# ActiveVisionLab/CrossScore

Measured on AMD Instinct MI355X. Metric: query-images/sec at 518x518, 5 ref views, bs=8; score-map MAE vs ref, higher is better.
Workload: dtype fp16

## Files before the change

### crossscore_amd/csrc/panel.hip

```cpp
#include "cs_common.h"
#include "panel_shared.h"
#include <atomic>
#include <stdlib.h>
#include <type_traits>
#include <utility>

namespace {

constexpr int PC = 384;
constexpr int PF = 1536;
constexpr int NT = PC / 32;
constexpr int KS = PC / 16;
constexpr int NSL = PF / 32;
constexpr int FRAG = 1024;
constexpr int CHUNK = 24 * FRAG;
constexpr int TICK = 48 * FRAG;
constexpr int OUT_CHUNKS = KS / 2;
constexpr int LAGT = 2;
constexpr int NTICK = NSL + LAGT;
constexpr int PAD_TICKS = 1;
constexpr int PANEL_ROWS = 128;
constexpr int LDS_RING = 0;
constexpr int LDS_X = 3 * CHUNK;
constexpr int XREC = 6 * FRAG;
constexpr int LDS_OF = LDS_X + 3 * 4 * 4 * FRAG;
constexpr int LDS_XF = 2 * TICK;
constexpr int LDS_HB = LDS_OF;
constexpr int HB_PAIR = 6 * FRAG;
constexpr int HB_RAW = 2 * FRAG;
constexpr int LDS_B1 = LDS_OF + 3 * 4 * 2 * FRAG;
constexpr int LDS_BV = LDS_B1 + PF * 4;
constexpr int LDS_BYTES = LDS_BV + 2 * PC * 4;
constexpr int ST_ROW = 784;
constexpr int ST_PAIR = 32 * ST_ROW;

#ifdef CS_PANEL_ABLATE
__device__ unsigned long long g_panel_dbg[64 * 8 * 16];
#define CS_STAMP(k) do { if (blockIdx.x < 64 && lane == 0) { \
    __builtin_amdgcn_sched_barrier(0); g_panel_dbg[(blockIdx.x * 8 + wv) * 16 + (k)] = __builtin_amdgcn_s_memtime(); __builtin_amdgcn_sched_barrier(0); } } while (0)
#define CS_STAMP_RT(k) do { if (blockIdx.x < 64 && lane == 0) g_panel_dbg[(blockIdx.x * 8 + wv) * 16 + (k)] = __builtin_amdgcn_s_memrealtime(); } while (0)
__device__ unsigned long long g_panel_bar[4 * 8 * 16 * 2];
#define CS_BAR_STAMP(v, k) do { if (blockIdx.x < 4 && (v) >= 40 && (v) < 56 && (threadIdx.x & 63) == 0) { \
    __builtin_amdgcn_sched_barrier(0); g_panel_bar[((blockIdx.x * 8 + wv) * 16 + ((v) - 40)) * 2 + (k)] = __builtin_amdgcn_s_memtime(); __builtin_amdgcn_sched_barrier(0); } } while (0)
#else
#define CS_STAMP(k) do { } while (0)
#define CS_STAMP_RT(k) do { } while (0)
#define CS_BAR_STAMP(v, k) do { } while (0)
#endif

template <bool OUTPROJ, int ABL = 0, bool BF = false>
__global__ __launch_bounds__(512, 2) void cs_panel_kernel(CsPanelParams p) {
  extern __shared__ __attribute__((aligned(16))) char smem[];
  const int tid = threadIdx.x;
  const int lane = tid & 63;
  const int wv = __builtin_amdgcn_readfirstlane(tid >> 6);
  const bool is_a = wv < 4;
  const int pair = wv & 3;
  const int j = lane & 31, h = lane >> 5;
  const int row0 = blockIdx.x * PANEL_ROWS + pair * 32;
  const size_t row = (size_t)min(row0 + j, p.M - 1);
  constexpr int NOUT = OUTPROJ ? OUT_CHUNKS : 0;
  constexpr size_t IMG_MLP = (size_t)NOUT * CHUNK;
  const unsigned lds0 = (unsigned)(size_t)CS_LDS_PTR(smem);
  const unsigned lane16 = lane * 16;
  const unsigned xoff = (unsigned)row * (PC * 4) + 64 * h;
  const unsigned ooff = (unsigned)row * (PC * 2) + 16 * h;

  int u_next = 0;
  auto out_unit_issue = [&](int c) {
    const int slot = c % 3;
    const unsigned dst = lds0 + LDS_RING + slot * CHUNK + pair * 6 * FRAG;
    const char* s6 = reinterpret_cast<const char*>(p.img) + (size_t)c * CHUNK + pair * 6 * FRAG + lane16;
    dma_piece<0>(s6, dst); dma_piece<FRAG>(s6, dst); dma_piece<2 * FRAG>(s6, dst); dma_piece<3 * FRAG>(s6, dst);
    dma_piece<0>(s6 + 4 * FRAG, dst + 4 * FRAG); dma_piece<FRAG>(s6 + 4 * FRAG, dst + 4 * FRAG);
    const unsigned dx = lds0 + LDS_X + (slot * 4 + pair) * XREC;
    const char* sx = reinterpret_cast<const char*>(p.x) + (size_t)(xoff + c * 128);
    dma_piece<0>(sx, dx); dma_piece<0>(sx + 16, dx + FRAG); dma_piece<0>(sx + 32, dx + 2 * FRAG); dma_piece<0>(sx + 48, dx + 3 * FRAG);
    const unsigned dof = dx + 4 * FRAG;
    const char* so = reinterpret_cast<const char*>(p.attn_o) + (size_t)(ooff + c * 64);
    dma_piece<0>(so, dof); dma_piece<0>(so + 32, dof + FRAG);
  };
  int pend_u = 0;
  bool pend = false;
  auto issue_piece = [&](auto K_) {
    constexpr int K = decltype(K_)::value;
    const unsigned dst = lds0 + LDS_RING + (pend_u & 3) * CHUNK + (pair * 6 + (K & ~3)) * FRAG;
    const char* s = reinterpret_cast<const char*>(p.img) + (IMG_MLP + (size_t)pend_u * CHUNK + (pair * 6 + (K & ~3)) * FRAG) + lane16;
    dma_piece<(K & 3) * FRAG>(s, dst);
  };
  auto tick_issue_all = [&](int t) {
    sfor<12>([&](auto K_) {
      constexpr int K = decltype(K_)::value % 6, HF = decltype(K_)::value / 6;
      const unsigned dst = lds0 + LDS_RING + (t & 1) * TICK + HF * CHUNK + (pair * 6 + (K & ~3)) * FRAG;
      const char* s = reinterpret_cast<const char*>(p.img) + (IMG_MLP + (size_t)t * TICK + HF * CHUNK + (pair * 6 + (K & ~3)) * FRAG) + lane16;
      dma_piece<(K & 3) * FRAG>(s, dst);
    });
  };
  unsigned long long tw_drain = 0, tw_vm = 0, tw_bar = 0;
  auto transition = [&](auto ISA_) -> unsigned {
    constexpr bool ISA = decltype(ISA_)::value;
    CS_SB();
    unsigned long long ta = 0, tb = 0, tc = 0, td = 0;
    if constexpr (ABL & 64) { asm volatile("s_memtime %0" : "=s"(ta)::"memory"); }
    asm volatile("s_waitcnt lgkmcnt(0)" ::: "memory");
    if constexpr (ABL & 64) { asm volatile("s_memtime %0\n\ts_waitcnt lgkmcnt(0)" : "=s"(tb)::"memory"); }
    if constexpr (ISA) {
      if (u_next + 1 < NOUT) CS_VMCNT(12);
      else CS_VMCNT(0);
    } else {
      CS_VMCNT(0);
    }
    if constexpr (ABL & 64) { asm volatile("s_memtime %0\n\ts_waitcnt lgkmcnt(0)" : "=s"(tc)::"memory"); }
    if constexpr (!(ABL & 16)) __builtin_amdgcn_s_barrier();
    if constexpr (ABL & 64) {
      asm volatile("s_memtime %0\n\ts_waitcnt lgkmcnt(0)" : "=s"(td)::"memory");
      tw_drain += tb - ta; tw_vm += tc - tb; tw_bar += td - tc;
    }
    asm volatile("" ::: "memory");
    if (u_next + 2 < NOUT) {
      if constexpr (ISA && OUTPROJ) out_unit_issue(u_next + 2);
    } else if (u_next + 1 >= NOUT) {
      const int t = u_next + 1 - NOUT;
      if constexpr (ISA) {
        if (t < 2) tick_issue_all(t);
      }
    }
    const unsigned base = lds0 + LDS_RING + lane16 + (u_next < NOUT ? (u_next % 3) * CHUNK : ((u_next - NOUT) & 1) * TICK);
    ++u_next;
    CS_SB();
    return base;
  };
  using TA = std::true_type;
  using TB = std::false_type;
  h16x8_t w[6];

  if (is_a) {
    CS_STAMP_RT(8); CS_STAMP(0);
    for (int i = tid; i < PF / 4; i += 256)
      reinterpret_cast<f32x4_t*>(smem + LDS_B1)[i] = reinterpret_cast<const f32x4_t*>(p.b1)[i];
    if (tid < PC / 4) {
      reinterpret_cast<f32x4_t*>(smem + LDS_BV)[tid] = OUTPROJ ? reinterpret_cast<const f32x4_t*>(p.bo)[tid] : f32x4_t{0.f, 0.f, 0.f, 0.f};
      reinterpret_cast<f32x4_t*>(smem + LDS_BV + PC * 4)[tid] = reinterpret_cast<const f32x4_t*>(p.b2)[tid];
    }
    asm volatile("s_waitcnt vmcnt(0) lgkmcnt(0)" ::: "memory");
    if constexpr (OUTPROJ) { out_unit_issue(0); out_unit_issue(1); }
    else tick_issue_all(0);
    unsigned cur = transition(TA{});
    CS_STAMP(1);
    for (int c = 0; c < NOUT; ++c) cur = transition(TA{});
    CS_STAMP(2);
    h16x8_t xf[KS];
    const unsigned r_addr = lds0 + LDS_XF + pair * 12 * FRAG + lane16;
    __builtin_amdgcn_s_barrier();
    sfor<12>([&](auto F_) { lds_read1<decltype(F_)::value * FRAG>(r_addr, xf[decltype(F_)::value]); });
    CS_LGKM(0);
    __builtin_amdgcn_s_barrier();
    __builtin_amdgcn_s_barrier();
    sfor<12>([&](auto F_) { lds_read1<decltype(F_)::value * FRAG>(r_addr, xf[12 + decltype(F_)::value]); });
    CS_LGKM(0);
    CS_STAMP(3);

    f32x16_t acE, acO;
    const unsigned bias_addr = lds0 + LDS_B1 + 64 * h;
    f32x4_t bb[4];
    auto read_bias = [&](int t) {
      const unsigned a = bias_addr + t * 128;
      lds_read_f4<0>(a, bb[0]); lds_read_f4<16>(a, bb[1]); lds_read_f4<32>(a, bb[2]); lds_read_f4<48>(a, bb[3]);
    };
    const unsigned hb_base = lds0 + LDS_HB + pair * HB_PAIR + lane16;
    const unsigned ring = lds0 + LDS_RING + lane16;
    unsigned xa[4] = {0u, 0u, 0u, 0u}, xb[4];
    PkGelu pg;
    const PkGeluK kk = pk_gelu_consts();
    auto boundary = [&](auto FC1_, int v) {
      CS_SB();
      if constexpr (!decltype(FC1_)::value) { asm volatile("s_waitcnt lgkmcnt(0)" ::: "memory"); }
      CS_BAR_STAMP(v, 0);
      CS_VMCNT(6);
      if constexpr (!(ABL & 16)) __builtin_amdgcn_s_barrier();
      asm volatile("" ::: "memory");
      CS_BAR_STAMP(v, 1);
      pend_u = v + 3;
      pend = v >= 1 && v + 3 < 2 * NTICK && !(ABL & 2);
      CS_SB();
    };
    auto tick = [&](auto FC1_, f32x16_t& acc, const f32x16_t& act, int hb_slot, int t, int t_next, bool hb_write) {
      constexpr bool FC1 = decltype(FC1_)::value;
      sfor<24>([&](auto M_) {
        constexpr int M = decltype(M_)::value;
        if constexpr (M == 6) boundary(FC1_, 2 * t);
        if constexpr (M == 18) {
          boundary(FC1_, 2 * t + 1);
          cur = ring + ((t + 1) & 1) * TICK;
          if constexpr (FC1) read_bias(t_next);
        }
        if constexpr ((M >= 6 && M < 12) || M >= 18) {
          if (pend) issue_piece(IC<(M >= 18 ? M - 18 : M - 6)>{});
        }
        if constexpr (M == 1) {
          if constexpr (!FC1) asm volatile("s_nop 15\n\ts_nop 15\n\ts_nop 15\n\ts_nop 15\n\ts_nop 15\n\ts_nop 15" ::: "memory");
#pragma unroll
          for (int i = 0; i < 4; ++i) xa[i] = pack_h16x2(act[2 * i], act[2 * i + 1]);
        }
        if constexpr (!BF) {
          if constexpr (M == 4) {
#pragma unroll
            for (int i = 0; i < 4; ++i) xb[i] = pack_h16x2(act[8 + 2 * i], act[9 + 2 * i]);
          }
          if constexpr (M == 5) {
            if (hb_write) lds_write16<HB_RAW>(hb_base + hb_slot * (2 * FRAG), u32x4_t{xb[0], xb[1], xb[2], xb[3]});
          }
        } else {
          if constexpr (M == 5) {
            if (hb_write) {
              lds_write16<HB_RAW>(hb_base + hb_slot * (2 * FRAG), __builtin_bit_cast(u32x4_t, f32x4_t{act[8], act[9], act[10], act[11]}));
              lds_write16<HB_RAW + FRAG>(hb_base + hb_slot * (2 * FRAG), __builtin_bit_cast(u32x4_t, f32x4_t{act[12], act[13], act[14], act[15]}));
            }
          }
        }
        if constexpr (FC1) {
          CS_LGKM(5);
          if constexpr (M == 0) {
            f32x16_t b16;
#pragma unroll
            for (int q = 0; q < 4; ++q)
#pragma unroll
              for (int i = 0; i < 4; ++i) b16[4 * q + i] = bb[q][i];
            if constexpr (ABL & 4) acc = b16;
            else acc = mfma_32x32x16<BF>(w[0], xf[0], b16);
          } else if constexpr (!(ABL & 4)) {
            acc = mfma_32x32x16<BF>(w[M % 6], xf[M], acc);
          }
          constexpr int F = (M + 6) % 24;
          if constexpr (!(ABL & 32)) lds_read1<((F / 12) * 24 + F % 12) * FRAG>(cur, w[M % 6]);
        }
        if constexpr (M >= 2 && M < 12 && !(ABL & 1)) {
          constexpr int B0 = M < 3 ? 0 : (M < 8 ? M - 1 : M);
          const float a8[8] = {act[0], act[1], act[2], act[3], act[4], act[5], act[6], act[7]};
          pk_gelu_op<B0, BF>(pg, xa, kk, a8);
          if constexpr (M == 2 || M == 7) pk_gelu_op<B0 + 1, BF>(pg, xa, kk, a8);
        }
        if constexpr (M == 11) { if (hb_write) lds_write16<0>(hb_base + hb_slot * FRAG, u32x4_t{xa[0], xa[1], xa[2], xa[3]}); }
        CS_SB();
      });
    };
    read_bias(0);
    sfor<6>([&](auto F_) { lds_read1<decltype(F_)::value * FRAG>(cur, w[decltype(F_)::value]); });
#pragma unroll
    for (int i = 0; i < 16; ++i) acO[i] = 0.f;
    for (int t = 0; t < NSL; t += 2) {
      tick(std::true_type{}, acE, acO, 1, t, t + 1, t > 0);
      tick(std::true_type{}, acO, acE, 0, t + 1, min(t + 2, NSL - 1), true);
    }
    CS_STAMP(4);
    CS_LGKM(0);
    tick(std::false_type{}, acE, acO, 1, NSL, 0, true);
    CS_VMCNT(0);
    if constexpr (!(ABL & 16)) __builtin_amdgcn_s_barrier();
    CS_STAMP(5);
    {
      const unsigned st_addr = lds0 + pair * ST_PAIR + (lane >> 4) * ST_ROW + (lane & 15) * 16;
      const int r_in = lane >> 4;
      auto drain = [&](char* gbase, size_t row_bytes) {
#pragma unroll
        for (int rg = 0; rg < 8; ++rg) {
          f32x4_t v[3];
          lds_read_f4<0>(st_addr + rg * 4 * ST_ROW, v[0]);
          lds_read_f4<256>(st_addr + rg * 4 * ST_ROW, v[1]);
          lds_read_f4<512>(st_addr + rg * 4 * ST_ROW, v[2]);
          CS_LGKM(0);
          const int r = rg * 4 + r_in;
          if (row0 + r < p.M) {
            char* g = gbase + (size_t)r * row_bytes + (lane & 15) * 16;
            *reinterpret_cast<f32x4_t*>(g) = v[0];
            *reinterpret_cast<f32x4_t*>(g + 256) = v[1];
            *reinterpret_cast<f32x4_t*>(g + 512) = v[2];
          }
        }
      };
      char* xg = reinterpret_cast<char*>(p.x + (size_t)row0 * PC);
      __builtin_amdgcn_s_barrier();
      __builtin_amdgcn_s_barrier();
      drain(xg, PC * 4);
      __builtin_amdgcn_s_barrier();
      __builtin_amdgcn_s_barrier();
      drain(xg + 768, PC * 4);
      __builtin_amdgcn_s_barrier();
      if (p.u_out) {
        __builtin_amdgcn_s_barrier();
        drain(reinterpret_cast<char*>(p.u_out + (size_t)row0 * PC), PC * 2);
      }
    }
    asm volatile("s_waitcnt vmcnt(0)" ::: "memory");
    CS_STAMP_RT(9);
#ifdef CS_PANEL_ABLATE
    if (blockIdx.x < 64 && lane == 0) { unsigned long long* d = g_panel_dbg + (blockIdx.x * 8 + wv) * 16; d[10] = tw_drain; d[11] = tw_vm; d[12] = tw_bar; }
#endif
    return;
  }

  CS_STAMP_RT(8); CS_STAMP(0);
  f32x16_t acc2[NT];
  const unsigned bv_addr = lds0 + LDS_BV + 64 * (fresh_lane() >> 5);
  unsigned cur = transition(TB{});
  CS_STAMP(1);
  auto add_bias = [&](auto T_, auto INIT_, int which) {
    constexpr int T = decltype(T_)::value;
    f32x4_t b4[4];
    const unsigned a = bv_addr + which * (PC * 4);
    lds_read_f4<T * 128>(a, b4[0]); lds_read_f4<T * 128 + 16>(a, b4[1]); lds_read_f4<T * 128 + 32>(a, b4[2]); lds_read_f4<T * 128 + 48>(a, b4[3]);
    CS_LGKM(0);
#pragma unroll
    for (int q = 0; q < 4; ++q)
#pragma unroll
      for (int i = 0; i < 4; ++i) acc2[T][4 * q + i] = (decltype(INIT_)::value ? 0.f : acc2[T][4 * q + i]) + b4[q][i];
  };
  if constexpr (OUTPROJ) {
    sfor<NT>([&](auto T_) { add_bias(T_, std::true_type{}, 0); });
    const unsigned xs_addr = lds0 + LDS_X + pair * XREC + lane16;
    h16x8_t of[2];
    lds_read1<4 * FRAG>(xs_addr, of[0]);
    lds_read1<5 * FRAG>(xs_addr, of[1]);
    sfor<6>([&](auto F_) { lds_read1<decltype(F_)::value * FRAG>(cur, w[decltype(F_)::value]); });
    int slot_x = 0;
    sfor<OUT_CHUNKS>([&](auto C_) {
      constexpr int C = decltype(C_)::value;
      f32x4_t xs;
      sfor<24>([&](auto M_) {
        constexpr int M = decltype(M_)::value;
        if constexpr (M >= 13 && M <= 16) {
          constexpr int Q = M - 13;
          CS_LGKM(1);
#pragma unroll
          for (int i = 0; i < 4; ++i) acc2[C][4 * Q + i] += xs[i];
          CS_SB();
        }
        if constexpr (M >= 12 && M <= 15) lds_read_f4<(M - 12) * FRAG>(xs_addr + slot_x * (4 * XREC), xs);
        if constexpr (M == 18) {
          cur = transition(TB{});
          slot_x = slot_x + 1 >= 3 ? 0 : slot_x + 1;
          if constexpr (C + 1 < OUT_CHUNKS) lds_read1<4 * FRAG>(xs_addr + slot_x * (4 * XREC), of[0]);
        }
        if constexpr (M == 0 && C > 0) lds_read1<5 * FRAG>(xs_addr + slot_x * (4 * XREC), of[1]);
        CS_LGKM(5);
        constexpr int T = M % 12;
        acc2[T] = mfma_32x32x16<BF>(w[M % 6], of[M / 12], acc2[T]);
        if constexpr (M < 18) lds_read1<(M + 6) * FRAG>(cur, w[M % 6]);
        else lds_read1<(M - 18) * FRAG>(cur, w[M % 6]);
        CS_SB();
      });
    });
    CS_LGKM(0);
  } else {
    const float* xr = p.x + row * PC + 16 * h;
#pragma unroll
    for (int T = 0; T < NT; ++T)
#pragma unroll
      for (int q = 0; q < 4; ++q) {
        const f32x4_t v = *reinterpret_cast<const f32x4_t*>(xr + 32 * T + 4 * q);
#pragma unroll
        for (int i = 0; i < 4; ++i) acc2[T][4 * q + i] = v[i];
      }
    asm volatile("s_waitcnt vmcnt(0)" ::: "memory");
  }
  CS_STAMP(2);

  auto row_stats = [&](float& mean, float& rstd) {
    float s = 0.f;
#pragma unroll
    for (int T = 0; T < NT; ++T)
#pragma unroll
      for (int r = 0; r < 16; r += 4) s += (acc2[T][r] + acc2[T][r + 1]) + (acc2[T][r + 2] + acc2[T][r + 3]);
    s = add_other_half(s);
    mean = s * (1.0f / PC);
    float q = 0.f;
#pragma unroll
    for (int T = 0; T < NT; ++T)
#pragma unroll
      for (int r = 0; r < 16; ++r) {
        const float d = acc2[T][r] - mean;
        q = fmaf(d, d, q);
      }
    q = add_other_half(q);
    rstd = 1.0f / sqrtf(q * (1.0f / PC) + p.eps);
  };
  {
    float mean, rstd;
    row_stats(mean, rstd);
    const float nb = -mean * rstd;
    const unsigned r_addr = lds0 + LDS_XF + pair * 12 * FRAG + lane16;
    auto put = [&](auto T_, auto S_) {
      constexpr int T = decltype(T_)::value, S = decltype(S_)::value;
      float v[8];
#pragma unroll
      for (int e = 0; e < 8; ++e) v[e] = fmaf(acc2[T][8 * S + e], rstd, nb);
      lds_write16<((2 * T + S) % 12) * FRAG>(r_addr, pack8<BF>(v));
    };
    sfor<6>([&](auto T_) { put(T_, IC<0>{}); put(T_, IC<1>{}); });
    asm volatile("s_waitcnt lgkmcnt(0)" ::: "memory");
    __builtin_amdgcn_s_barrier();
    __builtin_amdgcn_s_barrier();
    sfor<6>([&](auto T_) { put(IC<6 + decltype(T_)::value>{}, IC<0>{}); put(IC<6 + decltype(T_)::value>{}, IC<1>{}); });
    asm volatile("s_waitcnt lgkmcnt(0)" ::: "memory");
    __builtin_amdgcn_s_barrier();
  }
  sfor<NT>([&](auto T_) { add_bias(T_, std::false_type{}, 1); });
  CS_STAMP(3);

  for (int g = 0; g < 2 * LAGT; ++g) { if constexpr (!(ABL & 16)) __builtin_amdgcn_s_barrier(); }
  const unsigned hb_base = lds0 + LDS_HB + pair * HB_PAIR + lane16;
  int cur_step = TICK;
  h16x8_t hb0;
  u32x4_t hb1;
  f32x4_t rw[2];
  u32x4_t xr;
  unsigned hx[4];
  PkGelu pg;
  const PkGeluK kk = pk_gelu_consts();
  auto fc2_tick = [&](int slice, bool more) {
    sfor<24>([&](auto M_) {
      constexpr int M = decltype(M_)::value;
      if constexpr (M == 6) { CS_SB(); CS_BAR_STAMP(2 * (slice + LAGT), 0); if constexpr (!(ABL & 16)) __builtin_amdgcn_s_barrier(); asm volatile("" ::: "memory"); CS_BAR_STAMP(2 * (slice + LAGT), 1); CS_SB(); }
      if constexpr (M == 18) {
        if (more) {
          CS_SB();
          CS_BAR_STAMP(2 * (slice + LAGT) + 1, 0);
          if constexpr (!(ABL & 16)) __builtin_amdgcn_s_barrier();
          asm volatile("" ::: "memory");
          CS_BAR_STAMP(2 * (slice + LAGT) + 1, 1);
          cur += cur_step;
          cur_step = -cur_step;
          lds_read1<0>(hb_base + ((slice + 1) & 1) * FRAG, hb0);
          if constexpr (BF) {
            lds_read_f4<HB_RAW>(hb_base + ((slice + 1) & 1) * (2 * FRAG), rw[0]);
            lds_read_f4<HB_RAW + FRAG>(hb_base + ((slice + 1) & 1) * (2 * FRAG), rw[1]);
          } else {
            lds_read_u4<HB_RAW>(hb_base + ((slice + 1) & 1) * (2 * FRAG), xr);
          }
          CS_SB();
        }
      }
      CS_LGKM(5);
      if constexpr (ABL & 8) { if constexpr (M == 12) asm volatile("" ::"v"(hb1)); }
      else if constexpr (M < 12) acc2[M % 12] = mfma_32x32x16<BF>(w[M % 6], hb0, acc2[M % 12]);
      else acc2[M % 12] = mfma_32x32x16<BF>(w[M % 6], __builtin_bit_cast(h16x8_t, hb1), acc2[M % 12]);
      constexpr int F = (M + 6) % 24;
      if constexpr (!(ABL & 32)) lds_read1<((F / 12) * 24 + 12 + F % 12) * FRAG>(cur, w[M % 6]);
      if constexpr (M == 0) {
#pragma unroll
        for (int i = 0; i < 4; ++i) {
          if constexpr (BF) hx[i] = pack_h16x2(rw[i >> 1][2 * (i & 1)], rw[i >> 1][2 * (i & 1) + 1]);
          else hx[i] = xr[i];
        }
      }
      if constexpr (M < 12 && !(ABL & 1)) {
        const float a8[8] = {rw[0][0], rw[0][1], rw[0][2], rw[0][3], rw[1][0], rw[1][1], rw[1][2], rw[1][3]};
        pk_gelu_op<M, BF>(pg, hx, kk, a8);
      }
      if constexpr (M == 11) hb1 = u32x4_t{hx[0], hx[1], hx[2], hx[3]};
      CS_SB();
    });
  };
  cur = lds0 + LDS_RING + lane16;
  lds_read1<0>(hb_base, hb0);
  if constexpr (BF) {
    lds_read_f4<HB_RAW>(hb_base, rw[0]);
    lds_read_f4<HB_RAW + FRAG>(hb_base, rw[1]);
  } else {
    lds_read_u4<HB_RAW>(hb_base, xr);
  }
  sfor<6>([&](auto F_) { lds_read1<(12 + decltype(F_)::value) * FRAG>(cur, w[decltype(F_)::value]); });
  for (int sl = 0; sl < NSL - 1; ++sl) fc2_tick(sl, true);
  fc2_tick(NSL - 1, false);
  CS_LGKM(0);
  CS_VMCNT(0);
  CS_STAMP(4);

  {
    const unsigned le = fresh_lane();
    const unsigned st_addr = (unsigned)(size_t)CS_LDS_PTR(smem) + pair * ST_PAIR + (le & 31) * ST_ROW + 64 * (le >> 5);
    auto stage_x = [&](auto HALF_) {
      constexpr int HALF = decltype(HALF_)::value;
      sfor<6>([&](auto T_) {
        constexpr int T = 6 * HALF + decltype(T_)::value;
        sfor<4>([&](auto Q_) {
          constexpr int Q = decltype(Q_)::value;
          lds_write16<decltype(T_)::value * 128 + 16 * Q>(st_addr, __builtin_bit_cast(u32x4_t, f32x4_t{acc2[T][4 * Q], acc2[T][4 * Q + 1], acc2[T][4 * Q + 2], acc2[T][4 * Q + 3]}));
        });
      });
      asm volatile("s_waitcnt lgkmcnt(0)" ::: "memory");
    };
    __builtin_amdgcn_s_barrier();
    stage_x(IC<0>{});
    __builtin_amdgcn_s_barrier();
    float mean = 0.f, rstd = 0.f;
    if (p.u_out) row_stats(mean, rstd);
    __builtin_amdgcn_s_barrier();
    stage_x(IC<1>{});
    __builtin_amdgcn_s_barrier();
    __builtin_amdgcn_s_barrier();
    if (p.u_out) {
      const float nb = -mean * rstd;
      const unsigned su = (unsigned)(size_t)CS_LDS_PTR(smem) + pair * ST_PAIR + (le & 31) * ST_ROW + 32 * (le >> 5);
      sfor<NT>([&](auto T_) {
        constexpr int T = decltype(T_)::value;
        sfor<2>([&](auto Q_) {
          constexpr int Q = decltype(Q_)::value;
          float v[8];
#pragma unroll
          for (int e = 0; e < 8; ++e) v[e] = fmaf(acc2[T][8 * Q + e], rstd, nb);
          lds_write16<T * 64 + 16 * Q>(su, pack8<BF>(v));
        });
      });
      asm volatile("s_waitcnt lgkmcnt(0)" ::: "memory");
      __builtin_amdgcn_s_barrier();
    }
  }
  asm volatile("s_waitcnt vmcnt(0)" ::: "memory");
  CS_STAMP(5); CS_STAMP_RT(9);
#ifdef CS_PANEL_ABLATE
  if (blockIdx.x < 64 && lane == 0) { unsigned long long* d = g_panel_dbg + (blockIdx.x * 8 + wv) * 16; d[10] = tw_drain; d[11] = tw_vm; d[12] = tw_bar; }
#endif
}

__device__ __forceinline__ int panel_perm(int i) { return 16 * ((i >> 2) & 1) + (i & 3) + 4 * (i >> 3); }
template <bool BF>
__global__ __launch_bounds__(256) void cs_panel_pack_kernel(const float* __restrict__ wo, const float* __restrict__ ls1,
                                                            const float* __restrict__ w1, const float* __restrict__ g2,
                                                            const float* __restrict__ w2, const float* __restrict__ ls2,
                                                            h16_t* __restrict__ img) {
  const int nout = wo ? OUT_CHUNKS : 0;
  const long long n_out16 = (long long)nout * (CHUNK / 16);
  const long long total16 = n_out16 + (long long)(NTICK + PAD_TICKS) * (TICK / 16);
  const long long gi = (long long)blockIdx.x * blockDim.x + threadIdx.x;
  if (gi >= total16) return;
  float v[8] = {0.f, 0.f, 0.f, 0.f, 0.f, 0.f, 0.f, 0.f};
  if (gi < n_out16) {
    const int c = (int)(gi / (CHUNK / 16));
    const int within = (int)(gi - (long long)c * (CHUNK / 16));
    const int f = within >> 6, lane = within & 63, i = lane & 31, h = lane >> 5;
    const int ks = 2 * c + f / 12, T = f % 12;
    const int rowi = 32 * T + panel_perm(i);
#pragma unroll
    for (int e = 0; e < 8; ++e) v[e] = wo[(size_t)rowi * PC + 16 * ks + 8 * h + e] * (ls1 ? ls1[rowi] : 1.f);
  } else {
    const long long g2i = gi - n_out16;
    const int t = (int)(g2i / (TICK / 16));
    const int within = (int)(g2i - (long long)t * (TICK / 16));
    const int fpos = within >> 6, lane = within & 63, i = lane & 31, h = lane >> 5;
    const int f = ((fpos % 24) / 12) * 24 + (fpos / 24) * 12 + fpos % 12;
    if (t < NTICK) {
      if (f < 24) {
        if (t < NSL) {
          const int ks = f;
          const int rowi = 32 * t + panel_perm(i);
#pragma unroll
          for (int e = 0; e < 8; ++e) {
            const int col = 32 * (ks >> 1) + 16 * h + 8 * (ks & 1) + e;
            v[e] = w1[(size_t)rowi * PC + col] * (g2 ? g2[col] : 1.f);
          }
        }
      } else if (t >= LAGT) {
        const int tt = t - LAGT, fp = f - 24;
        const int s = fp / 12, T = fp % 12;
        const int rowi = 32 * T + panel_perm(i);
#pragma unroll
        for (int e = 0; e < 8; ++e) {
          const int col = 32 * tt + 16 * h + 8 * s + e;
          v[e] = w2[(size_t)rowi * PF + col] * (ls2 ? ls2[rowi] : 1.f);
        }
      }
    }
  }
  const uint4 o = {pack_o16x2<BF>(v[0], v[1]), pack_o16x2<BF>(v[2], v[3]), pack_o16x2<BF>(v[4], v[5]), pack_o16x2<BF>(v[6], v[7])};
  reinterpret_cast<uint4*>(img)[gi] = o;
}

template <bool OUTPROJ, bool BF>
hipError_t panel_launch_t(const CsPanelParams* p, hipStream_t st) {
  static std::atomic<bool> attr_done[16];
  int dev = 0;
  if (hipGetDevice(&dev) != hipSuccess || dev < 0 || dev >= 16) return hipErrorInvalidDevice;
  if (!attr_done[dev]) {
    hipError_t e = hipFuncSetAttribute(reinterpret_cast<const void*>(cs_panel_kernel<OUTPROJ, 0, BF>), hipFuncAttributeMaxDynamicSharedMemorySize, LDS_BYTES);
    if (e != hipSuccess) return e;
    attr_done[dev] = true;
  }
  const int grid = (p->M + PANEL_ROWS - 1) / PANEL_ROWS;
  hipLaunchKernelGGL((cs_panel_kernel<OUTPROJ, 0, BF>), dim3(grid), dim3(512), LDS_BYTES, st, *p);
  return hipGetLastError();
}

}

extern "C" {

#ifdef CS_PANEL_ABLATE
int cs_panel_debug_read(unsigned long long* dst) { return (int)hipMemcpyFromSymbol(dst, HIP_SYMBOL(g_panel_dbg), sizeof(g_panel_dbg)); }
int cs_panel_bar_read(unsigned long long* dst) { return (int)hipMemcpyFromSymbol(dst, HIP_SYMBOL(g_panel_bar), sizeof(g_panel_bar)); }
#endif

int cs_panel_supported(int C, int mlp_ratio) { return C == PC && mlp_ratio * C == PF; }
size_t cs_panel8_image_bytes(int with_outproj) { return (size_t)(with_outproj ? OUT_CHUNKS : 0) * CHUNK + (size_t)(NTICK + PAD_TICKS) * TICK; }

hipError_t cs_panel_pack_launch(const float* wo, const float* ls1, const float* w1, const float* g2, const float* w2, const float* ls2,
                                h16_t* img, int bf16, hipStream_t st) {
  const int total = (int)(cs_panel8_image_bytes(wo ? 1 : 0) / 16);
  if (bf16) hipLaunchKernelGGL(cs_panel_pack_kernel<true>, dim3((total + 255) / 256), dim3(256), 0, st, wo, ls1, w1, g2, w2, ls2, img);
  else hipLaunchKernelGGL(cs_panel_pack_kernel<false>, dim3((total + 255) / 256), dim3(256), 0, st, wo, ls1, w1, g2, w2, ls2, img);
  return hipGetLastError();
}

const char* cs_panel_check(const CsPanelParams* p) {
  if (!p->x || !p->img || !p->b1 || !p->b2) return "panel: null operand";
  if (p->attn_o && !p->bo) return "panel: the out-projection needs its bias";
  if (p->M <= 0) return "panel: empty shape";
  if ((long long)p->M * PC * 4 >= (1ll << 32)) return "panel: too many rows for 32-bit byte offsets";
  if (((uintptr_t)p->x | (uintptr_t)p->img | (uintptr_t)p->b1 | (uintptr_t)p->b2 | (uintptr_t)p->attn_o | (uintptr_t)p->u_out | (uintptr_t)p->bo) & 15)
    return "panel: operands must be 16-byte aligned";
  return nullptr;
}

hipError_t cs_panel_launch(const CsPanelParams* p, hipStream_t st) {
#ifdef CS_PANEL_ABLATE
  if (const char* e = getenv("CS_PANEL_ABL")) {
    const int abl = atoi(e);
    const int grid = (p->M + PANEL_ROWS - 1) / PANEL_ROWS;
#define CS_ABL_CASE(N) if (abl == N) { \
      (void)hipFuncSetAttribute(reinterpret_cast<const void*>(cs_panel_kernel<true, N>), hipFuncAttributeMaxDynamicSharedMemorySize, LDS_BYTES); \
      hipLaunchKernelGGL((cs_panel_kernel<true, N>), dim3(grid), dim3(512), LDS_BYTES, st, *p); return hipGetLastError(); }
    CS_ABL_CASE(1) CS_ABL_CASE(2) CS_ABL_CASE(3) CS_ABL_CASE(4) CS_ABL_CASE(8) CS_ABL_CASE(12) CS_ABL_CASE(16) CS_ABL_CASE(18) CS_ABL_CASE(32) CS_ABL_CASE(34) CS_ABL_CASE(50) CS_ABL_CASE(64)
#undef CS_ABL_CASE
  }
#endif
  if (p->attn_o) return p->bf16 ? panel_launch_t<true, true>(p, st) : panel_launch_t<true, false>(p, st);
  return p->bf16 ? panel_launch_t<false, true>(p, st) : panel_launch_t<false, false>(p, st);
}

}
```

### crossscore_amd/csrc/panel_shared.h

```cpp
#pragma once
#include "cs_common.h"
#include <type_traits>
#include <utility>

namespace {

constexpr int PANEL_FRAG = 1024;

#define CS_VMCNT(n) asm volatile("s_waitcnt vmcnt(%0)" ::"n"(n) : "memory")
#define CS_SB() __builtin_amdgcn_sched_barrier(0)
#define CS_LGKM(n) do { asm volatile("s_waitcnt lgkmcnt(%0)" ::"n"(n) : "memory"); CS_SB(); } while (0)

template <int V> using IC = std::integral_constant<int, V>;
template <int... Js, class F>
__device__ __forceinline__ void static_for(std::integer_sequence<int, Js...>, F&& f) {
  (f(IC<Js>{}), ...);
}
template <int N, class F>
__device__ __forceinline__ void sfor(F&& f) { static_for(std::make_integer_sequence<int, N>{}, f); }

struct PkGeluK { unsigned nk, c5, c4, c3, c2, c1, c0, vc6; };
__device__ __forceinline__ PkGeluK pk_gelu_consts() {
  PkGeluK k;
  asm volatile("s_mov_b32 %0, 0xb400b400" : "=s"(k.nk));
  asm volatile("s_mov_b32 %0, 0xbd76bd76" : "=s"(k.c5));
  asm volatile("s_mov_b32 %0, 0xb8a3b8a3" : "=s"(k.c4));
  asm volatile("s_mov_b32 %0, 0x3e8a3e8a" : "=s"(k.c3));
  asm volatile("s_mov_b32 %0, 0x394a394a" : "=s"(k.c2));
  asm volatile("s_mov_b32 %0, 0xb52cb52c" : "=s"(k.c1));
  asm volatile("s_mov_b32 %0, 0xb086b086" : "=s"(k.c0));
  asm volatile("v_mov_b32 %0, 0x3a443a44" : "=v"(k.vc6));
  return k;
}
struct PkGelu { unsigned t0, t1, q0, q1, r0, r1; };
template <int B, bool BF>
__device__ __forceinline__ void pk_gelu_block(PkGelu& g, unsigned& x0, unsigned& x1, const PkGeluK& k, float a0, float a1, float a2, float a3) {
  if constexpr (B == 0)
    asm("v_pk_max_f16 %0, %2, %2 neg_lo:[0,1] neg_hi:[0,1]\n\t"
        "v_pk_max_f16 %1, %3, %3 neg_lo:[0,1] neg_hi:[0,1]\n\t"
        "v_pk_fma_f16 %0, %0, %4, 1.0 op_sel_hi:[1,1,0] clamp\n\t"
        "v_pk_fma_f16 %1, %1, %4, 1.0 op_sel_hi:[1,1,0] clamp"
        : "=&v"(g.t0), "=&v"(g.t1) : "v"(x0), "v"(x1), "s"(k.nk));
  else if constexpr (B == 1)
    asm("v_pk_fma_f16 %0, %0, %0, -0.5 op_sel_hi:[1,1,0]\n\t"
        "v_pk_fma_f16 %1, %1, %1, -0.5 op_sel_hi:[1,1,0]\n\t"
        "v_pk_fma_f16 %2, %0, %4, %5\n\t"
        "v_pk_fma_f16 %3, %1, %4, %5"
        : "+v"(g.t0), "+v"(g.t1), "=&v"(g.q0), "=&v"(g.q1) : "v"(k.vc6), "s"(k.c5));
  else if constexpr (B == 2)
    asm("v_pk_fma_f16 %0, %0, %2, %4\n\t"
        "v_pk_fma_f16 %1, %1, %3, %4\n\t"
        "v_pk_fma_f16 %0, %0, %2, %5\n\t"
        "v_pk_fma_f16 %1, %1, %3, %5"
        : "+v"(g.q0), "+v"(g.q1) : "v"(g.t0), "v"(g.t1), "s"(k.c4), "s"(k.c3));
  else if constexpr (B == 3)
    asm("v_pk_fma_f16 %0, %0, %2, %4\n\t"
        "v_pk_fma_f16 %1, %1, %3, %4\n\t"
        "v_pk_fma_f16 %0, %0, %2, %5\n\t"
        "v_pk_fma_f16 %1, %1, %3, %5"
        : "+v"(g.q0), "+v"(g.q1) : "v"(g.t0), "v"(g.t1), "s"(k.c2), "s"(k.c1));
  else if constexpr (B == 4 && BF)
    asm("v_pk_fma_f16 %0, %0, %2, %4\n\t"
        "v_pk_fma_f16 %1, %1, %3, %4"
        : "+v"(g.q0), "+v"(g.q1) : "v"(g.t0), "v"(g.t1), "s"(k.c0));
  else if constexpr (B == 5 && BF) {
    float y0, y1, y2, y3;
    asm("v_max_f32 %2, 0, %6\n\t"
        "v_max_f32 %3, 0, %7\n\t"
        "v_max_f32 %4, 0, %8\n\t"
        "v_max_f32 %5, 0, %9\n\t"
        "v_fma_mix_f32 %2, %10, 1.0, %2 op_sel_hi:[1,0,0]\n\t"
        "v_fma_mix_f32 %3, %10, 1.0, %3 op_sel:[1,0,0] op_sel_hi:[1,0,0]\n\t"
        "v_fma_mix_f32 %4, %11, 1.0, %4 op_sel_hi:[1,0,0]\n\t"
        "v_fma_mix_f32 %5, %11, 1.0, %5 op_sel:[1,0,0] op_sel_hi:[1,0,0]\n\t"
        "v_cvt_pk_bf16_f32 %0, %2, %3\n\t"
        "v_cvt_pk_bf16_f32 %1, %4, %5"
        : "=&v"(x0), "=&v"(x1), "=&v"(y0), "=&v"(y1), "=&v"(y2), "=&v"(y3)
        : "v"(a0), "v"(a1), "v"(a2), "v"(a3), "v"(g.q0), "v"(g.q1));
  } else if constexpr (B == 4)
    asm("v_pk_fma_f16 %0, %0, %4, %6\n\t"
        "v_pk_fma_f16 %1, %1, %5, %6\n\t"
        "v_pk_max_f16 %2, %7, 0 op_sel_hi:[1,0]\n\t"
        "v_pk_max_f16 %3, %8, 0 op_sel_hi:[1,0]"
        : "+v"(g.q0), "+v"(g.q1), "=&v"(g.r0), "=&v"(g.r1) : "v"(g.t0), "v"(g.t1), "s"(k.c0), "v"(x0), "v"(x1));
  else
    asm("v_pk_add_f16 %0, %2, %4\n\t"
        "v_pk_add_f16 %1, %3, %5"
        : "=&v"(x0), "=&v"(x1) : "v"(g.q0), "v"(g.q1), "v"(g.r0), "v"(g.r1));
}
template <int N, bool BF>
__device__ __forceinline__ void pk_gelu_op(PkGelu& g, unsigned (&x)[4], const PkGeluK& k, const float (&a)[8]) {
  if constexpr (N >= 0 && N < 12) {
    constexpr int P = 2 * (N / 6);
    pk_gelu_block<N % 6, BF>(g, x[P], x[P + 1], k, a[2 * P], a[2 * P + 1], a[2 * P + 2], a[2 * P + 3]);
  }
}

__device__ __forceinline__ unsigned fresh_lane() {
  unsigned l;
  asm volatile("v_mbcnt_lo_u32_b32 %0, -1, 0\n\tv_mbcnt_hi_u32_b32 %0, -1, %0" : "=v"(l));
  return l;
}
__device__ __forceinline__ float add_other_half(float x) {
  const auto r = __builtin_amdgcn_permlane32_swap(__float_as_uint(x), __float_as_uint(x), false, false);
  return __uint_as_float(r[0]) + __uint_as_float(r[1]);
}

typedef unsigned u32x4_t __attribute__((ext_vector_type(4)));
template <bool BF>
__device__ __forceinline__ u32x4_t pack8(const float (&v)[8]) {
  return u32x4_t{pack_o16x2<BF>(v[0], v[1]), pack_o16x2<BF>(v[2], v[3]), pack_o16x2<BF>(v[4], v[5]), pack_o16x2<BF>(v[6], v[7])};
}

template <int OFF>
__device__ __forceinline__ void lds_read1(unsigned addr, h16x8_t& w) {
  asm volatile("ds_read_b128 %0, %1 offset:%2" : "=&v"(w) : "v"(addr), "n"(OFF) : "memory");
}
template <int OFF>
__device__ __forceinline__ void lds_read_f4(unsigned addr, f32x4_t& w) {
  asm volatile("ds_read_b128 %0, %1 offset:%2" : "=&v"(w) : "v"(addr), "n"(OFF) : "memory");
}
template <int OFF>
__device__ __forceinline__ void lds_read_u4(unsigned addr, u32x4_t& w) {
  asm volatile("ds_read_b128 %0, %1 offset:%2" : "=&v"(w) : "v"(addr), "n"(OFF) : "memory");
}
template <int OFF>
__device__ __forceinline__ void lds_write16(unsigned addr, u32x4_t v) {
  asm volatile("ds_write_b128 %0, %1 offset:%2" ::"v"(addr), "v"(v), "n"(OFF) : "memory");
}

template <int OFF>
__device__ __forceinline__ void dma_piece(const char* src, unsigned dst) {
  __builtin_amdgcn_global_load_lds(CS_GLOBAL_PTR(src), (__attribute__((address_space(3))) void*)(size_t)dst, 16, OFF, 0);
}


}
```

Baseline: 1381.

## Overlap bias preload with DMA and hand off LN output in one pass

Bias vectors are now loaded with asm global loads issued before the first DMA chunks and written to LDS after a partial vmcnt wait. Before, the code stalled on vmcnt(0) before any DMA was issued. The LN-normalized x is handed to the A waves in a single LDS pass instead of two halves, so LDS_XF moves and the second tick prefetch is deferred until after the x read. The bias add on acc2 is interleaved with the lag barriers, and the LN scale-shift uses a vector FMA. The risks are that the buffer placement now overlaps ring tick 1, and that the hand-tuned vmcnt counts may be wrong.

```diff
diff --git a/crossscore_amd/csrc/panel.hip b/crossscore_amd/csrc/panel.hip
--- a/crossscore_amd/csrc/panel.hip
+++ b/crossscore_amd/csrc/panel.hip
@@ -24,7 +24,7 @@
 constexpr int LDS_X = 3 * CHUNK;
 constexpr int XREC = 6 * FRAG;
 constexpr int LDS_OF = LDS_X + 3 * 4 * 4 * FRAG;
-constexpr int LDS_XF = 2 * TICK;
+constexpr int LDS_XF = TICK;
 constexpr int LDS_HB = LDS_OF;
 constexpr int HB_PAIR = 6 * FRAG;
 constexpr int HB_RAW = 2 * FRAG;
@@ -36,14 +36,18 @@
 
 #ifdef CS_PANEL_ABLATE
 __device__ unsigned long long g_panel_dbg[64 * 8 * 16];
-#define CS_STAMP(k) do { if (blockIdx.x < 64 && lane == 0) { \
-    __builtin_amdgcn_sched_barrier(0); g_panel_dbg[(blockIdx.x * 8 + wv) * 16 + (k)] = __builtin_amdgcn_s_memtime(); __builtin_amdgcn_sched_barrier(0); } } while (0)
-#define CS_STAMP_RT(k) do { if (blockIdx.x < 64 && lane == 0) g_panel_dbg[(blockIdx.x * 8 + wv) * 16 + (k)] = __builtin_amdgcn_s_memrealtime(); } while (0)
+#define CS_STAMP_DECL unsigned long long cs_t[6] = {0, 0, 0, 0, 0, 0}
+#define CS_STAMP(k) do { __builtin_amdgcn_sched_barrier(0); asm volatile("s_memtime %0\n\ts_waitcnt lgkmcnt(0)" : "=s"(cs_t[k]) :: "memory"); __builtin_amdgcn_sched_barrier(0); } while (0)
+#define CS_STAMP_DUMP do { if (blockIdx.x < 64 && fresh_lane() == 0) { unsigned long long* d = g_panel_dbg + (blockIdx.x * 8 + wv) * 16; \
+    d[0] = cs_t[0]; d[1] = cs_t[1]; d[2] = cs_t[2]; d[3] = cs_t[3]; d[4] = cs_t[4]; d[5] = cs_t[5]; d[10] = tw_drain; d[11] = tw_vm; d[12] = tw_bar; } } while (0)
+#define CS_STAMP_RT(k) do { if (blockIdx.x < 64 && fresh_lane() == 0) g_panel_dbg[(blockIdx.x * 8 + wv) * 16 + (k)] = __builtin_amdgcn_s_memrealtime(); } while (0)
 __device__ unsigned long long g_panel_bar[4 * 8 * 16 * 2];
 #define CS_BAR_STAMP(v, k) do { if (blockIdx.x < 4 && (v) >= 40 && (v) < 56 && (threadIdx.x & 63) == 0) { \
     __builtin_amdgcn_sched_barrier(0); g_panel_bar[((blockIdx.x * 8 + wv) * 16 + ((v) - 40)) * 2 + (k)] = __builtin_amdgcn_s_memtime(); __builtin_amdgcn_sched_barrier(0); } } while (0)
 #else
+#define CS_STAMP_DECL
 #define CS_STAMP(k) do { } while (0)
+#define CS_STAMP_DUMP do { } while (0)
 #define CS_STAMP_RT(k) do { } while (0)
 #define CS_BAR_STAMP(v, k) do { } while (0)
 #endif
@@ -96,6 +100,7 @@
       dma_piece<(K & 3) * FRAG>(s, dst);
     });
   };
+  CS_STAMP_DECL;
   unsigned long long tw_drain = 0, tw_vm = 0, tw_bar = 0;
   auto transition = [&](auto ISA_) -> unsigned {
     constexpr bool ISA = decltype(ISA_)::value;
@@ -122,7 +127,7 @@
     } else if (u_next + 1 >= NOUT) {
       const int t = u_next + 1 - NOUT;
       if constexpr (ISA) {
-        if (t < 2) tick_issue_all(t);
+        if (t == 0) tick_issue_all(t);
       }
     }
     const unsigned base = lds0 + LDS_RING + lane16 + (u_next < NOUT ? (u_next % 3) * CHUNK : ((u_next - NOUT) & 1) * TICK);
@@ -136,28 +141,37 @@
 
   if (is_a) {
     CS_STAMP_RT(8); CS_STAMP(0);
-    for (int i = tid; i < PF / 4; i += 256)
-      reinterpret_cast<f32x4_t*>(smem + LDS_B1)[i] = reinterpret_cast<const f32x4_t*>(p.b1)[i];
-    if (tid < PC / 4) {
-      reinterpret_cast<f32x4_t*>(smem + LDS_BV)[tid] = OUTPROJ ? reinterpret_cast<const f32x4_t*>(p.bo)[tid] : f32x4_t{0.f, 0.f, 0.f, 0.f};
-      reinterpret_cast<f32x4_t*>(smem + LDS_BV + PC * 4)[tid] = reinterpret_cast<const f32x4_t*>(p.b2)[tid];
-    }
-    asm volatile("s_waitcnt vmcnt(0) lgkmcnt(0)" ::: "memory");
+    const int tq = min(tid, PC / 4 - 1);
+    f32x4_t bq0, bq1, bq2 = {0.f, 0.f, 0.f, 0.f}, bq3;
+    global_read_f4(reinterpret_cast<const f32x4_t*>(p.b1) + tid, bq0);
+    global_read_f4(reinterpret_cast<const f32x4_t*>(p.b1) + 256 + (tid & 127), bq1);
+    if constexpr (OUTPROJ) global_read_f4(reinterpret_cast<const f32x4_t*>(p.bo) + tq, bq2);
+    global_read_f4(reinterpret_cast<const f32x4_t*>(p.b2) + tq, bq3);
     if constexpr (OUTPROJ) { out_unit_issue(0); out_unit_issue(1); }
     else tick_issue_all(0);
+    {
+      CS_SB();
+      CS_VMCNT(OUTPROJ ? 24 : 12);
+      CS_SB();
+      const unsigned bdst = lds0 + LDS_B1 + tid * 16;
+      lds_write16<0>(bdst, __builtin_bit_cast(u32x4_t, bq0));
+      if (tid < PF / 4 - 256) lds_write16<256 * 16>(bdst, __builtin_bit_cast(u32x4_t, bq1));
+      if (tid < PC / 4) {
+        lds_write16<LDS_BV - LDS_B1>(bdst, __builtin_bit_cast(u32x4_t, bq2));
+        lds_write16<LDS_BV - LDS_B1 + PC * 4>(bdst, __builtin_bit_cast(u32x4_t, bq3));
+      }
+    }
     unsigned cur = transition(TA{});
     CS_STAMP(1);
     for (int c = 0; c < NOUT; ++c) cur = transition(TA{});
     CS_STAMP(2);
     h16x8_t xf[KS];
-    const unsigned r_addr = lds0 + LDS_XF + pair * 12 * FRAG + lane16;
-    __builtin_amdgcn_s_barrier();
-    sfor<12>([&](auto F_) { lds_read1<decltype(F_)::value * FRAG>(r_addr, xf[decltype(F_)::value]); });
+    const unsigned r_addr = lds0 + LDS_XF + pair * KS * FRAG + lane16;
+    __builtin_amdgcn_s_barrier();
+    sfor<KS>([&](auto F_) { lds_read1<decltype(F_)::value * FRAG>(r_addr, xf[decltype(F_)::value]); });
     CS_LGKM(0);
     __builtin_amdgcn_s_barrier();
-    __builtin_amdgcn_s_barrier();
-    sfor<12>([&](auto F_) { lds_read1<decltype(F_)::value * FRAG>(r_addr, xf[12 + decltype(F_)::value]); });
-    CS_LGKM(0);
+    tick_issue_all(1);
     CS_STAMP(3);
 
     f32x16_t acE, acO;
@@ -176,7 +190,8 @@
       CS_SB();
       if constexpr (!decltype(FC1_)::value) { asm volatile("s_waitcnt lgkmcnt(0)" ::: "memory"); }
       CS_BAR_STAMP(v, 0);
-      CS_VMCNT(6);
+      if (v == 0) CS_VMCNT(12);
+      else CS_VMCNT(6);
       if constexpr (!(ABL & 16)) __builtin_amdgcn_s_barrier();
       asm volatile("" ::: "memory");
       CS_BAR_STAMP(v, 1);
@@ -293,9 +308,7 @@
     }
     asm volatile("s_waitcnt vmcnt(0)" ::: "memory");
     CS_STAMP_RT(9);
-#ifdef CS_PANEL_ABLATE
-    if (blockIdx.x < 64 && lane == 0) { unsigned long long* d = g_panel_dbg + (blockIdx.x * 8 + wv) * 16; d[10] = tw_drain; d[11] = tw_vm; d[12] = tw_bar; }
-#endif
+    CS_STAMP_DUMP;
     return;
   }
 
@@ -388,26 +401,38 @@
     float mean, rstd;
     row_stats(mean, rstd);
     const float nb = -mean * rstd;
-    const unsigned r_addr = lds0 + LDS_XF + pair * 12 * FRAG + lane16;
+    const unsigned r_addr = lds0 + LDS_XF + pair * KS * FRAG + lane16;
     auto put = [&](auto T_, auto S_) {
       constexpr int T = decltype(T_)::value, S = decltype(S_)::value;
-      float v[8];
-#pragma unroll
-      for (int e = 0; e < 8; ++e) v[e] = fmaf(acc2[T][8 * S + e], rstd, nb);
-      lds_write16<((2 * T + S) % 12) * FRAG>(r_addr, pack8<BF>(v));
+      const f32x16_t y = pk_fma(acc2[T], rstd, nb);
+      const float v[8] = {y[8 * S], y[8 * S + 1], y[8 * S + 2], y[8 * S + 3], y[8 * S + 4], y[8 * S + 5], y[8 * S + 6], y[8 * S + 7]};
+      lds_write16<(2 * T + S) * FRAG>(r_addr, pack8<BF>(v));
     };
-    sfor<6>([&](auto T_) { put(T_, IC<0>{}); put(T_, IC<1>{}); });
+    sfor<NT>([&](auto T_) { put(T_, IC<0>{}); put(T_, IC<1>{}); });
     asm volatile("s_waitcnt lgkmcnt(0)" ::: "memory");
     __builtin_amdgcn_s_barrier();
     __builtin_amdgcn_s_barrier();
-    sfor<6>([&](auto T_) { put(IC<6 + decltype(T_)::value>{}, IC<0>{}); put(IC<6 + decltype(T_)::value>{}, IC<1>{}); });
-    asm volatile("s_waitcnt lgkmcnt(0)" ::: "memory");
-    __builtin_amdgcn_s_barrier();
-  }
-  sfor<NT>([&](auto T_) { add_bias(T_, std::false_type{}, 1); });
+  }
   CS_STAMP(3);
 
-  for (int g = 0; g < 2 * LAGT; ++g) { if constexpr (!(ABL & 16)) __builtin_amdgcn_s_barrier(); }
+  sfor<2 * LAGT>([&](auto G_) {
+    constexpr int T0 = 3 * decltype(G_)::value;
+    f32x4_t b4[2][4];
+    const unsigned a = bv_addr + PC * 4;
+    sfor<4>([&](auto Q_) { lds_read_f4<T0 * 128 + 16 * decltype(Q_)::value>(a, b4[0][decltype(Q_)::value]); });
+    sfor<3>([&](auto I_) {
+      constexpr int I = decltype(I_)::value, T = T0 + I;
+      if constexpr (I < 2) sfor<4>([&](auto Q_) { lds_read_f4<(T + 1) * 128 + 16 * decltype(Q_)::value>(a, b4[(I + 1) & 1][decltype(Q_)::value]); });
+      sfor<4>([&](auto Q_) {
+        constexpr int Q = decltype(Q_)::value;
+        CS_LGKM((I < 2 ? 4 : 0) + 3 - Q);
+#pragma unroll
+        for (int i = 0; i < 4; ++i) acc2[T][4 * Q + i] += b4[I & 1][Q][i];
+      });
+      CS_SB();
+    });
+    if constexpr (!(ABL & 16)) __builtin_amdgcn_s_barrier();
+  });
   const unsigned hb_base = lds0 + LDS_HB + pair * HB_PAIR + lane16;
   int cur_step = TICK;
   h16x8_t hb0;
@@ -506,9 +531,8 @@
         constexpr int T = decltype(T_)::value;
         sfor<2>([&](auto Q_) {
           constexpr int Q = decltype(Q_)::value;
-          float v[8];
-#pragma unroll
-          for (int e = 0; e < 8; ++e) v[e] = fmaf(acc2[T][8 * Q + e], rstd, nb);
+          const f32x16_t y = pk_fma(acc2[T], rstd, nb);
+          const float v[8] = {y[8 * Q], y[8 * Q + 1], y[8 * Q + 2], y[8 * Q + 3], y[8 * Q + 4], y[8 * Q + 5], y[8 * Q + 6], y[8 * Q + 7]};
           lds_write16<T * 64 + 16 * Q>(su, pack8<BF>(v));
         });
       });
@@ -518,9 +542,7 @@
   }
   asm volatile("s_waitcnt vmcnt(0)" ::: "memory");
   CS_STAMP(5); CS_STAMP_RT(9);
-#ifdef CS_PANEL_ABLATE
-  if (blockIdx.x < 64 && lane == 0) { unsigned long long* d = g_panel_dbg + (blockIdx.x * 8 + wv) * 16; d[10] = tw_drain; d[11] = tw_vm; d[12] = tw_bar; }
-#endif
+  CS_STAMP_DUMP;
 }
 
 __device__ __forceinline__ int panel_perm(int i) { return 16 * ((i >> 2) & 1) + (i & 3) + 4 * (i >> 3); }
diff --git a/crossscore_amd/csrc/panel_shared.h b/crossscore_amd/csrc/panel_shared.h
--- a/crossscore_amd/csrc/panel_shared.h
+++ b/crossscore_amd/csrc/panel_shared.h
@@ -106,6 +106,20 @@
   return __uint_as_float(r[0]) + __uint_as_float(r[1]);
 }
 
+__device__ __forceinline__ f32x16_t pk_fma(const f32x16_t& a, float s, float b) {
+  f32x16_t r;
+#ifdef CS_PANEL_SCALAR_LN
+#pragma unroll
+  for (int i = 0; i < 16; ++i) r[i] = fmaf(a[i], s, b);
+#else
+  f32x16_t ss, bb;
+#pragma unroll
+  for (int i = 0; i < 16; ++i) { ss[i] = s; bb[i] = b; }
+  r = __builtin_elementwise_fma(a, ss, bb);
+#endif
+  return r;
+}
+
 typedef unsigned u32x4_t __attribute__((ext_vector_type(4)));
 template <bool BF>
 __device__ __forceinline__ u32x4_t pack8(const float (&v)[8]) {
@@ -124,6 +138,9 @@
 __device__ __forceinline__ void lds_read_u4(unsigned addr, u32x4_t& w) {
   asm volatile("ds_read_b128 %0, %1 offset:%2" : "=&v"(w) : "v"(addr), "n"(OFF) : "memory");
 }
+__device__ __forceinline__ void global_read_f4(const f32x4_t* src, f32x4_t& w) {
+  asm volatile("global_load_dwordx4 %0, %1, off" : "=&v"(w) : "v"(src) : "memory");
+}
 template <int OFF>
 __device__ __forceinline__ void lds_write16(unsigned addr, u32x4_t v) {
   asm volatile("ds_write_b128 %0, %1 offset:%2" ::"v"(addr), "v"(v), "n"(OFF) : "memory");
```

New measurement: 1384, median of 6. About the same (+0.2%).
